# vshmyhlo/retinanet-tensorflow

Hardware: AMD Instinct MI355X
Metric: train images/sec (MobileNetV2-FPN RetinaNet 512x512, bs=2/GPU) (higher is better)
Workload: dtype f32

## Files before the change

include/rn_hip.h:

```cpp
#ifndef RN_HIP_H
#define RN_HIP_H

#include <stddef.h>
#include <stdint.h>

#ifdef __cplusplus
extern "C" {
#endif

typedef void* rn_stream_t;

enum rn_status {
  RN_OK = 0,
  RN_EINVAL = -1,
  RN_EUNSUPPORTED = -2,
  RN_EHIP = -3,
  RN_EWORKSPACE = -4
};

enum rn_act { RN_ACT_NONE = 0, RN_ACT_RELU = 1, RN_ACT_ELU = 2, RN_ACT_RELU6 = 3, RN_ACT_SIGMOID = 4 };
enum rn_loss_mode { RN_LOSS_BCE_DICE = 0, RN_LOSS_FOCAL = 1 };
enum rn_opt { RN_OPT_MOMENTUM = 0, RN_OPT_RMSPROP = 1, RN_OPT_ADAM = 2 };

#define RN_MAX_SEG 16

typedef struct rn_reduce_list rn_reduce_list;

#define RN_API_VERSION 411
int rn_version(void);
const char* rn_last_error(void);

void rn_same_pad(int n, int k, int s, int* out, int* pad_before);

typedef struct rn_conv_seg {
  const float* x;
  const float* wgt;
  const float* bias;
  float* y;
  const float* dy;
  float* dx;
  int32_t n, h, w;
  int32_t cout;
  int32_t x_ld;
// ... 252 lines not shown
typedef struct rn_wino_gn {
  const float* in_rows;
  const float* in_gamma;
  const float* in_beta;
  int32_t in_groups, in_act;
  float in_eps;
  float* out_rows;
  int32_t out_groups;
  const void* u_ready;
  int32_t urot_ready;
} rn_wino_gn;
size_t rn_wino_gn_rows(const rn_conv_seg* segs, int nseg, int tile);
size_t rn_conv3x3_winograd_gn_u_bytes(int cin, int cout, int tile);
int rn_conv3x3_winograd_gn_weights(const float* w, int cin, int cout, int tile, void* u_out, size_t u_out_bytes, float* urot_out,
                                   rn_stream_t stream);
int rn_conv3x3_winograd_gn(const rn_conv_seg* segs, int nseg, int cin, int cout, const float* w, const float* bias, int tile,
                           const rn_wino_gn* gn, void* workspace, size_t workspace_bytes, float* v_buf, float* urot_buf,
                           rn_stream_t stream);
typedef struct rn_wino_gn_bwd {
  const float* in_rows;
  const float* in_gamma;
  const float* in_beta;
  int32_t in_groups, in_act;
  float in_eps;
  float* in_g_rows_group;
  float* in_g_rows_chan;
  const float* out_rows;
  const float* out_g_rows_group;
  const float* out_gamma;
  int32_t out_groups;
  float out_eps;
  int32_t defer_wgrad;
} rn_wino_gn_bwd;
int rn_conv3x3_winograd_gn_bwd(const rn_conv_seg* segs, int nseg, int cin, int cout, const float* w, float* dw, int accumulate,
                               int tile, const rn_wino_gn_bwd* gn, void* workspace, size_t workspace_bytes, const float* v_buf,
                               const float* urot_buf, rn_stream_t stream);
int rn_conv3x3_winograd_gn_bwd_wgrad(const rn_conv_seg* segs, int nseg, int cin, int cout, float* dw, int accumulate, int tile,
                                     void* workspace, size_t workspace_bytes, const float* v_buf, int urot_was_given, rn_stream_t stream);
int rn_reduce_rows(const float* in, float* out, int64_t count, int nrows, int accumulate, rn_stream_t stream, rn_reduce_list* defer);

typedef struct rn_mb_rows {
  float* rows;
  int32_t rows_per_sample, width, bn;
} rn_mb_rows;

typedef struct rn_mb_norm {
  const float* y;
  rn_mb_rows stat;
  float* mean; float* rstd;
  const float* gamma; const float* beta;
  int32_t c, groups, act;
  float eps, drop_rate;
  uint64_t drop_seed; const uint64_t* drop_seed_dev;
// ... 151 lines not shown
```

retinanet-tensorflow_amd/_rn.py:

```python
import ctypes as C
import os

import torch

_HERE = os.path.dirname(os.path.abspath(__file__))
LIB_PATH = os.environ.get("RN_LIB_PATH") or os.path.join(_HERE, "librn_hip.so")

MAX_SEG = 16
ACT = {None: 0, "none": 0, "linear": 0, "relu": 1, "elu": 2, "relu6": 3, "sigmoid": 4}
LOSS_MODE = {"bce_dice": 0, "focal": 1}
OPT = {"momentum": 0, "rmsprop": 1, "adam": 2}
OPT_BLOCK = 1024
LR_MAX_BOUNDARIES = 8
LOSS_STATS_HEADER = 8
API_VERSION = 411


class RnError(RuntimeError):
    pass


class LrSchedule(C.Structure):
    _fields_ = [("kind", C.c_int32), ("n_boundaries", C.c_int32), ("base_lr", C.c_double), ("warmup_factor", C.c_double),
                ("final_factor", C.c_double), ("decay_factor", C.c_double), ("warmup_steps", C.c_int64), ("total_steps", C.c_int64),
                ("boundaries", C.c_int64 * LR_MAX_BOUNDARIES)]


class ConvSeg(C.Structure):
    _fields_ = [("x", C.c_void_p), ("wgt", C.c_void_p), ("bias", C.c_void_p), ("y", C.c_void_p),
                ("dy", C.c_void_p), ("dx", C.c_void_p),
# ... 10 lines not shown
    _fields_ = [("kh", C.c_int32), ("kw", C.c_int32), ("stride", C.c_int32), ("cin", C.c_int32),
                ("groups", C.c_int32)]


class WinoGn(C.Structure):
    _fields_ = [("in_rows", C.c_void_p), ("in_gamma", C.c_void_p), ("in_beta", C.c_void_p), ("in_groups", C.c_int32),
                ("in_act", C.c_int32), ("in_eps", C.c_float), ("out_rows", C.c_void_p), ("out_groups", C.c_int32),
                ("u_ready", C.c_void_p), ("urot_ready", C.c_int32)]


class WinoGnBwd(C.Structure):
    _fields_ = [("in_rows", C.c_void_p), ("in_gamma", C.c_void_p), ("in_beta", C.c_void_p), ("in_groups", C.c_int32),
                ("in_act", C.c_int32), ("in_eps", C.c_float), ("in_g_rows_group", C.c_void_p), ("in_g_rows_chan", C.c_void_p),
                ("out_rows", C.c_void_p), ("out_g_rows_group", C.c_void_p), ("out_gamma", C.c_void_p),
                ("out_groups", C.c_int32), ("out_eps", C.c_float), ("defer_wgrad", C.c_int32)]


class ReduceDesc(C.Structure):
    _fields_ = [("in_", C.c_void_p), ("out", C.c_void_p), ("count", C.c_int32), ("nrows", C.c_uint16), ("accumulate", C.c_uint16)]


class ReduceList(C.Structure):
    _fields_ = [("desc", C.POINTER(ReduceDesc)), ("capacity", C.c_int32), ("count", C.c_int32)]

    @classmethod
    def make(cls, capacity=1024):
        arr = (ReduceDesc * capacity)()
        lst = cls(C.cast(arr, C.POINTER(ReduceDesc)), capacity, 0)
        lst._keep = arr
        return lst
# ... 94 lines not shown
    "rn_conv3x3_winograd_bwd_workspace", "rn_conv3x3_winograd_bwd", "rn_flush_reductions", "rn_gemm_batched",
    "rn_winograd_bwd_products_workspace", "rn_winograd_bwd_products", "rn_wino_gn_rows", "rn_conv3x3_winograd_gn", "rn_conv3x3_winograd_gn_bwd", "rn_conv3x3_winograd_gn_bwd_wgrad", "rn_reduce_rows", "rn_resize_bilinear_normalize", "rn_resize_pair_u8",
    "rn_resize_pair_u8_augment_workspace", "rn_resize_pair_u8_augment",
    "rn_resize_pair_u8_batch", "rn_resize_pair_u8_augment_batch_workspace", "rn_resize_pair_u8_augment_batch",
    "rn_dwgn_supported", "rn_dwgn_fwd", "rn_dwgn_bwd", "rn_depthwise_fwd", "rn_depthwise_dgrad", "rn_depthwise_wgrad_workspace", "rn_depthwise_wgrad", "rn_depthwise_bwd",
    "rn_group_norm_sync_bytes", "rn_group_norm_workspace", "rn_group_norm_fwd", "rn_group_norm_bwd",
    "rn_act_fwd", "rn_act_bwd", "rn_upsample_add_fwd", "rn_upsample_add_bwd_top",
    "rn_pack_weights_f16", "rn_pack_weights_f16_bytes", "rn_cast_f32_to_f16", "rn_pad_cast_rgb_f16", "rn_conv2d_fwd_f16", "rn_conv2d_f16_fold_rows", "rn_conv2d_fwd_f16_fold", "rn_group_norm_finalize", "rn_group_norm_apply_f16", "rn_group_norm_apply_res_f16", "rn_maxpool_fwd_f16", "rn_maxpool_gn_fwd_f16", "rn_upsample_add_fwd_f16",
    "rn_act_fwd_f16", "rn_flip_width", "rn_dropout", "rn_dropout_strided", "rn_maxpool_fwd", "rn_maxpool_bwd", "rn_maxpool_bwd_arg", "rn_avgpool_fwd", "rn_avgpool_bwd",
    "rn_loss_workspace", "rn_loss_fwd", "rn_loss_bwd",
    "rn_iou", "rn_anchor_assign", "rn_anchor_assign_levels", "rn_anchor_assign_levels_pair", "rn_decode_boxes", "rn_detect_workspace", "rn_detect",
    "rn_boxes_decode", "rn_nms_classwise_workspace", "rn_nms_classwise",
    "rn_optimizer_workspace", "rn_grad_norm_l2reg", "rn_optimizer_step", "rn_counter_add", "rn_add_segs",
    "rn_mb_rows_max", "rn_mb_compact_rows_layout", "rn_mb_compact_rows", "rn_mb_pointwise_rows", "rn_mb_pointwise_fwd", "rn_mb_depthwise_rows", "rn_mb_depthwise_fwd", "rn_mb_apply",
    "rn_mb_resident_sync_bytes", "rn_mb_resident_rows", "rn_mb_resident_fwd", "rn_set_product_mode", "rn_get_product_mode",
    "rn_set_x3_bfrag", "rn_get_x3_bfrag", "rn_x3_bfrag_ok", "rn_x3_bfrag_bytes", "rn_x3_pack_bfrag", "rn_gemm_batched_bfrag", "rn_conv3x3_winograd_gn_u_bytes", "rn_conv3x3_winograd_gn_weights",
    "rn_conv2d_f16_stats_tiles", "rn_group_norm_fwd_f16_tiles",
    "rn_mb_pointwise_bwd_rows", "rn_mb_pointwise_bwd_workspace", "rn_mb_pointwise_bwd",
    "rn_mb_depthwise_bwd_rows", "rn_mb_depthwise_bwd_workspace", "rn_mb_depthwise_bwd",
    "rn_debug_collective_standin", "rn_optimizer_norm_pairs", "rn_optimizer_step_norm", "rn_norm_reg_finalize",
    "rn_lr_schedule_eval", "rn_optimizer_step_norm_lrdev",
]


def lib():
    global _lib
    if _lib is None:
        if not os.path.exists(LIB_PATH):
            raise RnError("librn_hip.so not found at %s: build it with "
                          "`make -C retinanet-tensorflow_amd/csrc` (there is no fallback path)" % LIB_PATH)
        L = C.CDLL(LIB_PATH)
# ... 68 lines not shown
        L.rn_conv3x3_winograd_bwd_workspace.argtypes = [C.c_void_p] + [C.c_int] * 6
        L.rn_conv3x3_winograd_bwd.argtypes = [C.c_void_p, C.c_int, C.c_int, C.c_int, C.c_void_p, C.c_void_p, C.c_int, C.c_int,
                                              C.c_void_p, C.c_size_t, C.c_void_p, C.c_void_p, C.c_void_p]
        L.rn_conv3x3_winograd_keep_bytes.argtypes = [C.c_void_p, C.c_int, C.c_int, C.c_int, C.c_int, C.c_void_p, C.c_void_p]
        L.rn_conv3x3_winograd.argtypes = [C.c_void_p, C.c_int, C.c_int, C.c_int, C.c_void_p, C.c_void_p, C.c_int, C.c_int,
                                          C.c_void_p, C.c_size_t, C.c_void_p, C.c_void_p, C.c_void_p]
        L.rn_wino_gn_rows.argtypes = [C.c_void_p, C.c_int, C.c_int]
        L.rn_winograd_bwd_products_workspace.argtypes = [C.c_int] * 4
        L.rn_winograd_bwd_products.argtypes = [C.c_void_p] * 3 + [C.c_int] * 3 + [C.c_void_p] * 2 + [C.c_int] * 3 + \
                                              [C.c_void_p, C.c_size_t, C.c_void_p, C.c_void_p]
        L.rn_x3_bfrag_ok.argtypes = [C.c_int] * 3
        L.rn_conv2d_f16_stats_tiles.argtypes = [C.c_void_p, C.c_int, C.c_void_p, C.c_void_p]
        L.rn_group_norm_fwd_f16_tiles.argtypes = [C.c_void_p, C.c_int, C.c_void_p, C.c_void_p, C.c_void_p, C.c_void_p, C.c_void_p, C.c_void_p]
        L.rn_conv3x3_winograd_gn_u_bytes.argtypes = [C.c_int] * 3
        L.rn_conv3x3_winograd_gn_weights.argtypes = [C.c_void_p, C.c_int, C.c_int, C.c_int, C.c_void_p, C.c_size_t, C.c_void_p, C.c_void_p]
        L.rn_x3_bfrag_bytes.argtypes = [C.c_int] * 3
        L.rn_x3_pack_bfrag.argtypes = [C.c_void_p, C.c_void_p] + [C.c_int] * 4 + [C.c_void_p]
        L.rn_gemm_batched_bfrag.argtypes = [C.c_void_p] * 3 + [C.c_int] * 5 + [C.c_void_p]
        L.rn_set_x3_bfrag.argtypes = [C.c_int]
        L.rn_conv3x3_winograd_gn.argtypes = [C.c_void_p, C.c_int, C.c_int, C.c_int, C.c_void_p, C.c_void_p, C.c_int, C.c_void_p,
                                             C.c_void_p, C.c_size_t, C.c_void_p, C.c_void_p, C.c_void_p]
        L.rn_conv3x3_winograd_gn_bwd_wgrad.argtypes = [C.c_void_p, C.c_int, C.c_int, C.c_int, C.c_void_p, C.c_int, C.c_int, C.c_void_p, C.c_size_t,
                                                       C.c_void_p, C.c_int, C.c_void_p]
        L.rn_conv3x3_winograd_gn_bwd.argtypes = [C.c_void_p, C.c_int, C.c_int, C.c_int, C.c_void_p, C.c_void_p, C.c_int, C.c_int,
                                                 C.c_void_p, C.c_void_p, C.c_size_t, C.c_void_p, C.c_void_p, C.c_void_p]
        L.rn_reduce_rows.argtypes = [C.c_void_p, C.c_void_p, C.c_int64, C.c_int, C.c_int, C.c_void_p, C.c_void_p]
        L.rn_conv2d_bias_grad.argtypes = [C.c_void_p, C.c_int, C.c_void_p, C.c_void_p, C.c_void_p, C.c_size_t,
                                          C.c_void_p, C.c_void_p]
        L.rn_group_norm_workspace.argtypes = [C.c_void_p, C.c_int, C.c_void_p]
        L.rn_group_norm_fwd.argtypes = [C.c_void_p, C.c_int, C.c_void_p, C.c_void_p, C.c_void_p, C.c_void_p,
                                        C.c_size_t, C.c_void_p]
        L.rn_group_norm_bwd.argtypes = [C.c_void_p, C.c_int, C.c_void_p, C.c_void_p, C.c_void_p, C.c_void_p,
                                        C.c_void_p, C.c_void_p, C.c_size_t, C.c_void_p, C.c_void_p]
        L.rn_act_fwd.argtypes = [C.c_void_p, C.c_void_p, C.c_int64, C.c_int, C.c_void_p]
        L.rn_act_bwd.argtypes = [C.c_void_p, C.c_void_p, C.c_void_p, C.c_int64, C.c_int, C.c_void_p]
        L.rn_upsample_add_fwd.argtypes = [C.c_void_p] * 3 + [C.c_int] * 6 + [C.c_void_p]
        L.rn_upsample_add_bwd_top.argtypes = [C.c_void_p] * 2 + [C.c_int] * 6 + [C.c_void_p]
        L.rn_pack_weights_f16.argtypes = [C.c_void_p, C.c_void_p, C.c_int, C.c_int, C.c_int, C.c_int, C.c_void_p]
# ... 225 lines not shown
```

retinanet-tensorflow_amd/csrc/winograd.hip:

```cpp
#include "rn_common.h"

namespace {
constexpr int NT = 256;

struct WSeg { const float* x; float* y; int n, h, w, th, tw, tile_start; };
struct WArgs {
  WSeg seg[RN_MAX_SEG];
  int nseg, c, total_tiles;
  float* buf;
  const float* bias;
};

__device__ __forceinline__ int seg_of_tile(const WArgs& a, int t) {
  int s = 0;
  while (s + 1 < a.nseg && t >= a.seg[s + 1].tile_start) ++s;
  return s;
}

template <int W>
struct VecW { typedef float type __attribute__((ext_vector_type(W))); };
template <>
struct VecW<1> { typedef float type; };

template <int M>
// ... 332 lines not shown
__host__ __device__ inline int weight_blocks_f32(const WeightArgs& wa) { return (wa.u || wa.u2) ? (int)((wa.kn + NT - 1) / NT) : 0; }
__host__ __device__ inline int weight_blocks_frag(const WeightArgs& wa) {
  return wa.uf ? (int)(((int64_t)(wa.cin / 2) * ((wa.cout + 31) / 32) * 32 + NT - 1) / NT) : 0;
}
__host__ __device__ inline int weight_blocks(const WeightArgs& wa) { return weight_blocks_f32(wa) + weight_blocks_frag(wa); }
template <int M>
__device__ __forceinline__ void wino_weight_any_body(const WeightArgs& wa, int blk) {
  const int n0 = weight_blocks_f32(wa);
  if (blk < n0) wino_weight_body<M>(wa.w, wa.u, wa.u2, wa.kn, wa.rot, blk);
  else wino_weight_frag_body<M>(wa.w, wa.uf, wa.cin, wa.cout, blk - n0);
}

template <int M>
__global__ __launch_bounds__(NT) void wino_weight_any_kernel(const WeightArgs wa) {
  wino_weight_any_body<M>(wa, blockIdx.x);
}

template <int M>
__global__ __launch_bounds__(NT) void wino_dw_kernel(const float* __restrict__ du, float* __restrict__ dw, int64_t kn, int nsplit,
                                                    int accumulate) {
  wino_dw_body<M>(du, dw, kn, nsplit, accumulate, blockIdx.x);
}
template <int M>
__global__ __launch_bounds__(NT) void wino_weight_kernel(const float* __restrict__ w, float* __restrict__ u, float* __restrict__ u2,
                                                        int64_t kn, int rot) {
  wino_weight_body<M>(w, u, u2, kn, rot, blockIdx.x);
}

struct DwArgs2 { const float* du; float* dw; int64_t kn; int nsplit, accumulate; };

// ... 760 lines not shown
template <int M, int W, template <int> class LT>
__global__ __launch_bounds__(chunk_threads<W>()) void wino_gn_input_kernel(const CArgs in, const Fold f, int slabs) {
  chunk_input_body<M, W, LT>(in, f, blockIdx.x / slabs, blockIdx.x % slabs);
}
template <int M, int W>
__global__ __launch_bounds__(chunk_threads<W>()) void wino_gn_output_kernel(const CArgs out, const Fold f, int slabs) {
  chunk_output_body<M, W, 0>(out, f, blockIdx.x / slabs, blockIdx.x % slabs);
}
template <int M, int W, template <int> class LT>
__global__ __launch_bounds__(chunk_threads<W>(), chunk_waves<W>()) void wino_gn_bwd_pre_kernel(const CArgs dgrad_in, const CArgs wgrad_dy, const Fold f,
                                                                               int nb_first, int slabs) {
  const int b = blockIdx.x;
  if (b < nb_first) chunk_input_body<M, W, LT>(dgrad_in, f, b / slabs, b % slabs);
  else chunk_dy_body<M, W, LT>(wgrad_dy, f, (b - nb_first) / slabs, (b - nb_first) % slabs);
}
template <int M, int W, int MODE>
__global__ __launch_bounds__(chunk_threads<W>(), chunk_waves<W>()) void wino_gn_bwd_post_kernel(const CArgs out, const Fold f, const DwArgs2 d, int nb_out,
                                                                                int slabs) {
  const int b = blockIdx.x;
  if (b < nb_out) chunk_output_body<M, W, MODE>(out, f, b / slabs, b % slabs);
  else wino_dw_body<M>(d.du, d.dw, d.kn, d.nsplit, d.accumulate, b - nb_out);
}

int cfill(const rn_conv_seg* segs, int nseg, int c, int m, CArgs* a, const float* const* xs, const float* const* auxs, float* const* ys) {
  int64_t tiles = 0, chunks = 0;
  for (int s = 0; s < nseg; ++s) {
    CSeg& d = a->seg[s];
    d.n = segs[s].n; d.h = segs[s].h; d.w = segs[s].w;
    d.th = (d.h + m - 1) / m; d.tw = (d.w + m - 1) / m;
    d.tile_start = (int)tiles; d.chunk_start = (int)chunks;
// ... 17 lines not shown
  return 2;
}
}

extern "C" size_t rn_wino_gn_rows(const rn_conv_seg* segs, int nseg, int tile) {
  if (!segs || nseg < 1 || nseg > RN_MAX_SEG || (tile != 2 && tile != 4)) return 0;
  size_t chunks = 0;
  for (int s = 0; s < nseg; ++s) {
    const size_t tps = (size_t)((segs[s].h + tile - 1) / tile) * ((segs[s].w + tile - 1) / tile);
    chunks += (size_t)segs[s].n * ((tps + CK_TILES - 1) / CK_TILES);
  }
  return chunks;
}

namespace {
#define RN_WGN(W_, CALL)                          \
  do {                                            \
    if (W_ == 4) { constexpr int W = 4; CALL; }   \
    else if (W_ == 2) { constexpr int W = 2; CALL; } \
    else { constexpr int W = 1; CALL; }           \
  } while (0)

template <int M>
int run_gn_fwd(const rn_conv_seg* segs, int nseg, int cin, int cout, const float* w, const float* bias, const rn_wino_gn* gn, float* U,
               float* V, float* Mb, float* v_buf, float* urot_buf, hipStream_t st) {
  constexpr int P2 = (M + 2) * (M + 2);
  const float* xs[RN_MAX_SEG]; float* ys[RN_MAX_SEG];
  for (int s = 0; s < nseg; ++s) { xs[s] = segs[s].x; ys[s] = segs[s].y; }
  CArgs ia = {}, oa = {};
  cfill(segs, nseg, cin, M, &ia, xs, nullptr, nullptr);
// ... 72 lines not shown
    fi.rows = gn->in_rows; fi.gamma = gn->in_gamma; fi.beta = gn->in_beta; fi.groups = gn->in_groups; fi.cpg = cin / gn->in_groups;
    fi.act = gn->in_act; fi.eps = gn->in_eps; fi.g_rows_group = gn->in_g_rows_group; fi.g_rows_chan = gn->in_g_rows_chan;
  }
  const int wi = chunk_width(T_, cin, fold_in ? fi.cpg : 0);
  if (!V) {
    CArgs xa = {};
    cfill(segs, nseg, cin, M, &xa, xins, nullptr, nullptr);
    xa.buf = (float*)(ws + L.v);
    const int slabs = cin / (CK_LANES * wi);
    if (fold_in) RN_WGN(wi, hipLaunchKernelGGL((wino_gn_input_kernel<M, W, LoadGnAct>), dim3(xa.total_chunks * slabs), dim3(chunk_threads<W>()), 0, st, xa, fi, slabs));
    else RN_WGN(wi, hipLaunchKernelGGL((wino_gn_input_kernel<M, W, LoadPlain>), dim3(xa.total_chunks * slabs), dim3(chunk_threads<W>()), 0, st, xa, fi, slabs));
    V = xa.buf;
  }
  ia.buf = Vdy;
  ya.buf = dM;
  if (fold_out) {
    Fold fo = {};
    fo.rows = gn->out_rows; fo.grows = gn->out_g_rows_group; fo.gamma = gn->out_gamma; fo.groups = gn->out_groups;
    fo.cpg = cout / gn->out_groups; fo.eps = gn->out_eps;
    const int wy = chunk_width(T_, cout, fo.cpg);
    const int slabs = cout / (CK_LANES * wy), nb = ia.total_chunks * slabs;
    RN_WGN(wy, hipLaunchKernelGGL((wino_gn_bwd_pre_kernel<M, W, LoadGnBwd>), dim3(2 * nb), dim3(chunk_threads<W>()), 0, st, ia, ya, fo, nb, slabs));
  } else {
    WArgs wia = {}, woa = {}, wya = {}, unused = {};
    if (int e = fill(segs, nseg, cin, cout, M, true, &wia, &woa, true)) return e;
    if (int e = fill(segs, nseg, cin, cout, M, true, &wya, &unused, true)) return e;
    wia.buf = Vdy; wya.buf = dM;
    const int wy = width_for(T_, cout);
    const int nb = (int)grid_for((int64_t)T_ * cout / wy);
    if (wy == 4) hipLaunchKernelGGL((wino_bwd_pre_kernel<M, 4>), dim3(2 * nb), dim3(NT), 0, st, wia, wya, nb);
    else if (wy == 2) hipLaunchKernelGGL((wino_bwd_pre_kernel<M, 2>), dim3(2 * nb), dim3(NT), 0, st, wia, wya, nb);
    else hipLaunchKernelGGL((wino_bwd_pre_kernel<M, 1>), dim3(2 * nb), dim3(NT), 0, st, wia, wya, nb);
  }
  RN_LAUNCH_CHECK();
  int nsplit = 1;
  const bool defer = gn->defer_wgrad != 0;
  if (defer) {
    if (int e = rn::launch_batched_gemm(Vdy, Urot, Mdx, T_, cout, cin, P2, 1, st)) return e;
  } else if (int e = rn::launch_winograd_bwd_products(Vdy, Urot, Mdx, T_, cout, cin, V, dM, cin, cout, P2, ws + L.slab, ws_bytes - L.slab, st,
                                                      &nsplit)) {
    return e;
  }
  oa.buf = Mdx; oa.bias = nullptr;
  {
    const DwArgs2 d = {(const float*)(ws + L.slab), dw, kn, nsplit, accumulate};
    const int slabs = cin / (CK_LANES * wi), nb_out = oa.total_chunks * slabs, nb_dw = defer ? 0 : (int)rn::ceil_div64(kn, NT);
    if (!fold_in) { fi.groups = 1; fi.cpg = CK_LANES * wi; }
    if (fold_in) RN_WGN(wi, hipLaunchKernelGGL((wino_gn_bwd_post_kernel<M, W, 1>), dim3(nb_out + nb_dw), dim3(chunk_threads<W>()), 0, st, oa, fi, d, nb_out, slabs));
    else RN_WGN(wi, hipLaunchKernelGGL((wino_gn_bwd_post_kernel<M, W, 0>), dim3(nb_out + nb_dw), dim3(chunk_threads<W>()), 0, st, oa, fi, d, nb_out, slabs));
  }
  RN_LAUNCH_CHECK();
  return RN_OK;
}
#undef RN_WGN

template <int M>
int run_gn_bwd_wgrad(const rn_conv_seg* segs, int nseg, int cin, int cout, float* dw, int accumulate, char* ws, const BwdLayout& L,
                     size_t ws_bytes, const float* v_buf, hipStream_t st) {
  constexpr int P2 = (M + 2) * (M + 2);
  const int T_ = (int)tiles_of(segs, nseg, M);
  const int64_t kn = (int64_t)cin * cout;
  const float* V = v_buf ? v_buf : (const float*)(ws + L.v);
  const float* dM = (const float*)(ws + L.dm);
  int nsplit = 1;
  if (int e = rn::launch_batched_gemm_tn(V, dM, nullptr, T_, cin, cout, P2, ws + L.slab, ws_bytes - L.slab, st, &nsplit, 1)) return e;
  hipLaunchKernelGGL(wino_dw_kernel<M>, dim3((unsigned)rn::ceil_div64(kn, NT)), dim3(NT), 0, st, (const float*)(ws + L.slab), dw, kn, nsplit,
                     accumulate);
  RN_LAUNCH_CHECK();
  return RN_OK;
}

int check_fold(const rn_conv_seg* segs, int nseg, int cin, int cout, int tile) {
  RN_CHECK_ARG(segs && nseg >= 1 && nseg <= RN_MAX_SEG && (tile == 2 || tile == 4), "winograd gn: bad segments / tile");
  RN_UNSUPPORTED(cin % CK_MAXCH != 0 || cout % 4 != 0, "winograd gn: cin %d must be a multiple of %d, cout %d of 4", cin, CK_MAXCH, cout);
  for (int s = 0; s < nseg; ++s) {
    RN_CHECK_ARG(segs[s].n >= 1 && segs[s].h >= 1 && segs[s].w >= 1, "winograd gn: bad segment %d", s);
    RN_UNSUPPORTED((double)segs[s].n * segs[s].h * segs[s].w * (cin > cout ? cin : cout) * 4.0 >= 2147483648.0,
                   "winograd gn: segment %d >= 2 GiB", s);
  }
  return RN_OK;
}
}

extern "C" size_t rn_conv3x3_winograd_gn_u_bytes(int cin, int cout, int tile) {
  if (cin < 1 || cout < 1 || (tile != 2 && tile != 4)) return 0;
  return u_bytes((size_t)(tile + 2) * (tile + 2), cin, cout);
}
extern "C" int rn_conv3x3_winograd_gn_weights(const float* w, int cin, int cout, int tile, void* u_out, size_t u_out_bytes, float* urot_out,
                                              rn_stream_t stream) {
  RN_CHECK_ARG(w && u_out && (tile == 2 || tile == 4), "winograd gn weights: bad argument");
  RN_UNSUPPORTED(cin % CK_MAXCH != 0 || cout % 4 != 0, "winograd gn weights: cin %d must be a multiple of %d, cout %d of 4", cin, CK_MAXCH, cout);
  const size_t need = rn_conv3x3_winograd_gn_u_bytes(cin, cout, tile);
  if (u_out_bytes < need) {
    rn::set_error("winograd gn weights: u_out %zu < %zu bytes", u_out_bytes, need);
    return RN_EWORKSPACE;
  }
  const bool u_frag = rn::x3_bfrag_format(cin, cout);
  const WeightArgs wa = {w, u_frag ? nullptr : (float*)u_out, urot_out, (int64_t)cin * cout, 0, u_frag ? (unsigned*)u_out : nullptr, cin, cout};
  hipStream_t st = (hipStream_t)stream;
  if (tile == 2) hipLaunchKernelGGL(wino_weight_any_kernel<2>, dim3((unsigned)weight_blocks(wa)), dim3(NT), 0, st, wa);
  else hipLaunchKernelGGL(wino_weight_any_kernel<4>, dim3((unsigned)weight_blocks(wa)), dim3(NT), 0, st, wa);
  RN_LAUNCH_CHECK();
  return RN_OK;
}

extern "C" int rn_conv3x3_winograd_gn_bwd_wgrad(const rn_conv_seg* segs, int nseg, int cin, int cout, float* dw, int accumulate, int tile,
                                                void* workspace, size_t workspace_bytes, const float* v_buf, int urot_was_given,
                                                rn_stream_t stream) {
  if (int e = check_fold(segs, nseg, cin, cout, tile)) return e;
  RN_CHECK_ARG(dw && workspace, "winograd gn bwd wgrad: null pointer");
  const BwdLayout L = bwd_layout(segs, nseg, cin, cout, tile, v_buf == nullptr, urot_was_given == 0);
  if (workspace_bytes < L.total) {
    rn::set_error("winograd gn bwd wgrad: workspace %zu < %zu bytes", workspace_bytes, L.total);
    return RN_EWORKSPACE;
  }
  hipStream_t st = (hipStream_t)stream;
  return tile == 2 ? run_gn_bwd_wgrad<2>(segs, nseg, cin, cout, dw, accumulate, (char*)workspace, L, workspace_bytes, v_buf, st)
                   : run_gn_bwd_wgrad<4>(segs, nseg, cin, cout, dw, accumulate, (char*)workspace, L, workspace_bytes, v_buf, st);
}

extern "C" int rn_conv3x3_winograd_gn(const rn_conv_seg* segs, int nseg, int cin, int cout, const float* w, const float* bias, int tile,
                                      const rn_wino_gn* gn, void* workspace, size_t workspace_bytes, float* v_buf, float* urot_buf,
                                      rn_stream_t stream) {
  if (int e = check_fold(segs, nseg, cin, cout, tile)) return e;
  RN_CHECK_ARG(w && workspace && gn, "winograd gn: null pointer");
  for (int s = 0; s < nseg; ++s) RN_CHECK_ARG(segs[s].x && segs[s].y, "winograd gn: null tensor in segment %d", s);
  if (gn->in_rows) {
    RN_CHECK_ARG(gn->in_gamma && gn->in_beta, "winograd gn: null gamma / beta");
    RN_UNSUPPORTED(!fold_ok(cin, gn->in_groups), "winograd gn: %d channels in %d groups cannot be folded", cin, gn->in_groups);
  }
  if (gn->out_rows) RN_UNSUPPORTED(!fold_ok(cout, gn->out_groups), "winograd gn: %d channels in %d groups cannot be folded", cout, gn->out_groups);
  const size_t need = rn_conv3x3_winograd_workspace(segs, nseg, cin, cout, tile);
  if (workspace_bytes < need) {
// ... 3 lines not shown
  const size_t p2 = (size_t)(tile + 2) * (tile + 2), tiles = tiles_of(segs, nseg, tile);
  RN_UNSUPPORTED((double)tiles * (cin > cout ? cin : cout) * 4.0 >= 2147483648.0, "winograd gn: a transform plane is >= 2 GiB");
  float* U = (float*)workspace;
  float* V = (float*)((char*)workspace + rn::align_up(u_bytes(p2, cin, cout), 256));
  float* Mb = (float*)((char*)V + rn::align_up(p2 * tiles * cin * 4, 256));
  hipStream_t st = (hipStream_t)stream;
  return tile == 2 ? run_gn_fwd<2>(segs, nseg, cin, cout, w, bias, gn, U, V, Mb, v_buf, urot_buf, st)
                   : run_gn_fwd<4>(segs, nseg, cin, cout, w, bias, gn, U, V, Mb, v_buf, urot_buf, st);
}

extern "C" int rn_conv3x3_winograd_gn_bwd(const rn_conv_seg* segs, int nseg, int cin, int cout, const float* w, float* dw, int accumulate,
                                          int tile, const rn_wino_gn_bwd* gn, void* workspace, size_t workspace_bytes, const float* v_buf,
                                          const float* urot_buf, rn_stream_t stream) {
  if (int e = check_fold(segs, nseg, cin, cout, tile)) return e;
  RN_CHECK_ARG(w && dw && workspace && gn, "winograd gn bwd: null pointer");
  for (int s = 0; s < nseg; ++s) RN_CHECK_ARG(segs[s].x && segs[s].dy && segs[s].dx, "winograd gn bwd: null tensor in segment %d", s);
  if (gn->in_rows) {
    RN_CHECK_ARG(gn->in_gamma && gn->in_beta && gn->in_g_rows_group && gn->in_g_rows_chan, "winograd gn bwd: null input-side pointer");
    RN_UNSUPPORTED(!fold_ok(cin, gn->in_groups), "winograd gn bwd: %d channels in %d groups cannot be folded", cin, gn->in_groups);
  }
  if (gn->out_rows) {
    RN_CHECK_ARG(gn->out_g_rows_group && gn->out_gamma, "winograd gn bwd: null output-side pointer");
    for (int s = 0; s < nseg; ++s) RN_CHECK_ARG(segs[s].y, "winograd gn bwd: the folded output side needs the raw conv output y (segment %d)", s);
    RN_UNSUPPORTED(!fold_ok(cout, gn->out_groups), "winograd gn bwd: %d channels in %d groups cannot be folded", cout, gn->out_groups);
  }
  const BwdLayout L = bwd_layout(segs, nseg, cin, cout, tile, v_buf == nullptr, urot_buf == nullptr);
  if (workspace_bytes < L.total) {
    rn::set_error("winograd gn bwd: workspace %zu < %zu bytes", workspace_bytes, L.total);
    return RN_EWORKSPACE;
  }
// ... 5 lines not shown
```

retinanet-tensorflow_amd/ops.py:

```python
import ctypes as C
import os

import torch

import _rn


DIRECT_PARAM_GRADS = False


WGRAD_SIDE_STREAM = False


class _on_side_stream(object):

    def __init__(self, device, tensors, direct=True):
        self.on = WGRAD_SIDE_STREAM and direct and device.type == 'cuda'
        if self.on:
            self.side = _rn.side_stream(device, 0)
            self.side.wait_stream(torch.cuda.current_stream(device))
            for t in tensors:
                if t is not None:
                    t.record_stream(self.side)
            self.ctx = torch.cuda.stream(self.side)
# ... 418 lines not shown
    for w, gamma, beta in tower:
        kh, kw, ci, co = w.shape
        g = gn_groups(co, groups)
        if not (kh == 3 and kw == 3 and ci == cin and ci % 64 == 0 and co % 64 == 0 and 64 % (co // g) == 0):
            return False
        cin = co
    if out_w is not None and not (out_w.shape[0] == 3 and out_w.shape[1] == 3 and out_w.shape[2] == cin and out_w.shape[3] % 4 == 0):
        return False
    m = WINOGRAD_TILE
    tiles = sum(x.shape[0] * ((x.shape[1] + m - 1) // m) * ((x.shape[2] + m - 1) // m) for x in xs)
    widest = max([cin] + [t[0].shape[3] for t in tower] + ([out_w.shape[3]] if out_w is not None else []))
    return 4 * (m + 2) ** 2 * (tiles * 2 * widest + widest * widest) <= WINOGRAD_MAX_WORKSPACE


WINO_PRE = {}


class WinoPretransform(object):

    def __init__(self, weights):
        L = _rn.lib()
        self.items = []
        for w in weights:
            cin, cout = int(w.shape[2]), int(w.shape[3])
            ub = int(L.rn_conv3x3_winograd_gn_u_bytes(cin, cout, WINOGRAD_TILE))
            u = torch.empty((ub + 3) // 4, dtype=torch.float32, device=w.device)
            urot = torch.empty((WINOGRAD_TILE + 2) ** 2 * cin * cout, dtype=torch.float32, device=w.device)
            self.items.append((w, u, urot))

    def launch(self):
        L = _rn.lib()
        for w, u, urot in self.items:
            _rn.check(L.rn_conv3x3_winograd_gn_weights(_rn.f32(w), int(w.shape[2]), int(w.shape[3]), WINOGRAD_TILE, u.data_ptr(), u.numel() * 4,
                                                       _rn.f32(urot), _rn.stream()), "rn_conv3x3_winograd_gn_weights")
        ev = torch.cuda.Event()
        ev.record(torch.cuda.current_stream())
        return {w.data_ptr(): (u, urot, ev) for w, u, urot in self.items}, ev


class _WinoTower(torch.autograd.Function):

    @staticmethod
    def forward(ctx, cfg, n, *args):
        groups, eps, act, k, with_out = cfg
        xs = [x.contiguous() for x in args[:n]]
        params = list(args[n:])
        tower = [(params[3 * i], params[3 * i + 1], params[3 * i + 2]) for i in range(k)]
        out_w, out_b = (params[3 * k], params[3 * k + 1]) if with_out else (None, None)
        L = _rn.lib()
# ... 87 lines not shown
                gnb.in_rows, gnb.in_gamma, gnb.in_beta = ctx.rows[i - 1].data_ptr(), _rn.f32(gamma), _rn.f32(beta)
                gnb.in_groups, gnb.in_act, gnb.in_eps = g_in, _rn.ACT[act], eps
                gnb.in_g_rows_group, gnb.in_g_rows_chan = grg.data_ptr(), grc.data_ptr()
            if i < nfold:
                _, gamma_o, _b = tower[i]
                for j in range(n):
                    segs[j].y = _rn.f32(inputs[i + 1][j])
                gnb.out_rows, gnb.out_g_rows_group = ctx.rows[i].data_ptr(), g_rows_group_next.data_ptr()
                gnb.out_gamma, gnb.out_groups, gnb.out_eps = _rn.f32(gamma_o), gn_groups(cout, groups), eps
            v_buf, u_buf = ctx.keep[i]
            dw_buf, dw = _grad_slot(w)
            need = L.rn_conv3x3_winograd_bwd_workspace(segs, n, cin, cout, tile, 1 if v_buf is not None else 0,
                                                       1 if u_buf is not None else 0)
            defer = WGRAD_DEFER is not None and dw is None
            ws = torch.empty(int(need), dtype=torch.uint8, device=dev) if defer else _rn.workspace(need, dev)
            gnb.defer_wgrad = 1 if defer else 0
            _rn.check(L.rn_conv3x3_winograd_gn_bwd(segs, n, cin, cout, _rn.f32(w), _rn.f32(dw_buf), 0, tile, C.byref(gnb),
                                                   ws.data_ptr(), ws.numel(),
                                                   _rn.f32(v_buf) if v_buf is not None else None,
                                                   _rn.f32(u_buf) if u_buf is not None else None, _rn.stream()),
                      "rn_conv3x3_winograd_gn_bwd")
            if defer:
                WGRAD_DEFER.append((segs, n, cin, cout, dw_buf, tile, ws, v_buf, 1 if u_buf is not None else 0, x_in))
            grads[3 * i if i < k else 3 * k] = dw
            if i == nconv - 1 and out_b is not None and ctx.needs_input_grad[2 + n + 3 * k + 1]:
                db_buf, db = _grad_slot(out_b)
                geom = _rn.ConvGeom(3, 3, 1, cin, 1)
                need = L.rn_conv2d_bias_grad_workspace(cout)
                wsb = _grad_workspace(need, dev)
                _rn.check(L.rn_conv2d_bias_grad(segs, n, C.byref(geom), _rn.f32(db_buf), wsb.data_ptr(), wsb.numel(), _rn.stream(), _defer_arg()),
                          "rn_conv2d_bias_grad")
                grads[3 * k + 1] = db
            if i > 0:
                _, gamma, beta = tower[i - 1]
                dg_buf, dg = _grad_slot(gamma)
                db_buf, db = _grad_slot(beta)
                if _deferring:
                    _deferred_keep.append(grc)
                _rn.check(L.rn_reduce_rows(_rn.f32(grc[0]), _rn.f32(db_buf), cin, ctx.nrows, 0, _rn.stream(), _defer_arg()), "rn_reduce_rows")
                _rn.check(L.rn_reduce_rows(_rn.f32(grc[1]), _rn.f32(dg_buf), cin, ctx.nrows, 0, _rn.stream(), _defer_arg()), "rn_reduce_rows")
                grads[3 * (i - 1) + 1], grads[3 * (i - 1) + 2] = dg, db
            cur_dy = dxs
            g_rows_group_next = grg
        return (None, None) + tuple(cur_dy) + tuple(grads)


WGRAD_DEFER = None


def run_deferred_wgrads(records):
    L = _rn.lib()
    for segs, n, cin, cout, dw_buf, tile, ws, v_buf, urot_given, _keep in records:
        _rn.check(L.rn_conv3x3_winograd_gn_bwd_wgrad(segs, n, cin, cout, _rn.f32(dw_buf), 0, tile, ws.data_ptr(), ws.numel(),
                                                     _rn.f32(v_buf) if v_buf is not None else None, urot_given, _rn.stream()),
                  "rn_conv3x3_winograd_gn_bwd_wgrad")


def wino_tower(xs, tower, out_w=None, out_b=None, groups=32, eps=1e-5, act=None):
    k = len(tower)
    cfg = (groups, float(eps), act, k, out_w is not None)
    flat = [t for layer in tower for t in layer]
    if out_w is not None:
        flat += [out_w, out_b]
    return list(_WinoTower.apply(cfg, len(xs), *xs, *flat))


class _Depthwise(torch.autograd.Function):

    @staticmethod
# ... 696 lines not shown
```

Measured before the change: 479.8.

## Batch winograd weight pretransforms into one launch; optionally defer dy transform to wgrad

New measurement: 480.5 (median of 3 runs). No clear change (+0.2%).

```diff
diff --git a/include/rn_hip.h b/include/rn_hip.h
--- a/include/rn_hip.h
+++ b/include/rn_hip.h
@@ -26,7 +26,7 @@
 
 typedef struct rn_reduce_list rn_reduce_list;
 
-#define RN_API_VERSION 411
+#define RN_API_VERSION 412
 int rn_version(void);
 const char* rn_last_error(void);
 
@@ -309,6 +309,15 @@
 size_t rn_conv3x3_winograd_gn_u_bytes(int cin, int cout, int tile);
 int rn_conv3x3_winograd_gn_weights(const float* w, int cin, int cout, int tile, void* u_out, size_t u_out_bytes, float* urot_out,
                                    rn_stream_t stream);
+#define RN_WINO_MAX_KERNELS 16
+typedef struct rn_wino_kernel {
+  const float* w;
+  int32_t cin, cout;
+  void* u_out;
+  size_t u_out_bytes;
+  float* urot_out;
+} rn_wino_kernel;
+int rn_conv3x3_winograd_gn_weights_many(const rn_wino_kernel* kernels, int nkernels, int tile, int max_blocks, rn_stream_t stream);
 int rn_conv3x3_winograd_gn(const rn_conv_seg* segs, int nseg, int cin, int cout, const float* w, const float* bias, int tile,
                            const rn_wino_gn* gn, void* workspace, size_t workspace_bytes, float* v_buf, float* urot_buf,
                            rn_stream_t stream);
@@ -331,7 +340,8 @@
                                int tile, const rn_wino_gn_bwd* gn, void* workspace, size_t workspace_bytes, const float* v_buf,
                                const float* urot_buf, rn_stream_t stream);
 int rn_conv3x3_winograd_gn_bwd_wgrad(const rn_conv_seg* segs, int nseg, int cin, int cout, float* dw, int accumulate, int tile,
-                                     void* workspace, size_t workspace_bytes, const float* v_buf, int urot_was_given, rn_stream_t stream);
+                                     void* workspace, size_t workspace_bytes, const float* v_buf, int urot_was_given,
+                                     const rn_wino_gn_bwd* gn, rn_stream_t stream);
 int rn_reduce_rows(const float* in, float* out, int64_t count, int nrows, int accumulate, rn_stream_t stream, rn_reduce_list* defer);
 
 typedef struct rn_mb_rows {
diff --git a/retinanet-tensorflow_amd/_rn.py b/retinanet-tensorflow_amd/_rn.py
--- a/retinanet-tensorflow_amd/_rn.py
+++ b/retinanet-tensorflow_amd/_rn.py
@@ -13,7 +13,7 @@
 OPT_BLOCK = 1024
 LR_MAX_BOUNDARIES = 8
 LOSS_STATS_HEADER = 8
-API_VERSION = 411
+API_VERSION = 412
 
 
 class RnError(RuntimeError):
@@ -54,6 +54,14 @@
                 ("in_act", C.c_int32), ("in_eps", C.c_float), ("in_g_rows_group", C.c_void_p), ("in_g_rows_chan", C.c_void_p),
                 ("out_rows", C.c_void_p), ("out_g_rows_group", C.c_void_p), ("out_gamma", C.c_void_p),
                 ("out_groups", C.c_int32), ("out_eps", C.c_float), ("defer_wgrad", C.c_int32)]
+
+
+WINO_MAX_KERNELS = 16
+
+
+class WinoKernel(C.Structure):
+    _fields_ = [("w", C.c_void_p), ("cin", C.c_int32), ("cout", C.c_int32), ("u_out", C.c_void_p), ("u_out_bytes", C.c_size_t),
+                ("urot_out", C.c_void_p)]
 
 
 class ReduceDesc(C.Structure):
@@ -178,7 +186,7 @@
     "rn_optimizer_workspace", "rn_grad_norm_l2reg", "rn_optimizer_step", "rn_counter_add", "rn_add_segs",
     "rn_mb_rows_max", "rn_mb_compact_rows_layout", "rn_mb_compact_rows", "rn_mb_pointwise_rows", "rn_mb_pointwise_fwd", "rn_mb_depthwise_rows", "rn_mb_depthwise_fwd", "rn_mb_apply",
     "rn_mb_resident_sync_bytes", "rn_mb_resident_rows", "rn_mb_resident_fwd", "rn_set_product_mode", "rn_get_product_mode",
-    "rn_set_x3_bfrag", "rn_get_x3_bfrag", "rn_x3_bfrag_ok", "rn_x3_bfrag_bytes", "rn_x3_pack_bfrag", "rn_gemm_batched_bfrag", "rn_conv3x3_winograd_gn_u_bytes", "rn_conv3x3_winograd_gn_weights",
+    "rn_set_x3_bfrag", "rn_get_x3_bfrag", "rn_x3_bfrag_ok", "rn_x3_bfrag_bytes", "rn_x3_pack_bfrag", "rn_gemm_batched_bfrag", "rn_conv3x3_winograd_gn_u_bytes", "rn_conv3x3_winograd_gn_weights", "rn_conv3x3_winograd_gn_weights_many",
     "rn_conv2d_f16_stats_tiles", "rn_group_norm_fwd_f16_tiles",
     "rn_mb_pointwise_bwd_rows", "rn_mb_pointwise_bwd_workspace", "rn_mb_pointwise_bwd",
     "rn_mb_depthwise_bwd_rows", "rn_mb_depthwise_bwd_workspace", "rn_mb_depthwise_bwd",
@@ -277,6 +285,7 @@
         L.rn_group_norm_fwd_f16_tiles.argtypes = [C.c_void_p, C.c_int, C.c_void_p, C.c_void_p, C.c_void_p, C.c_void_p, C.c_void_p, C.c_void_p]
         L.rn_conv3x3_winograd_gn_u_bytes.argtypes = [C.c_int] * 3
         L.rn_conv3x3_winograd_gn_weights.argtypes = [C.c_void_p, C.c_int, C.c_int, C.c_int, C.c_void_p, C.c_size_t, C.c_void_p, C.c_void_p]
+        L.rn_conv3x3_winograd_gn_weights_many.argtypes = [C.c_void_p, C.c_int, C.c_int, C.c_int, C.c_void_p]
         L.rn_x3_bfrag_bytes.argtypes = [C.c_int] * 3
         L.rn_x3_pack_bfrag.argtypes = [C.c_void_p, C.c_void_p] + [C.c_int] * 4 + [C.c_void_p]
         L.rn_gemm_batched_bfrag.argtypes = [C.c_void_p] * 3 + [C.c_int] * 5 + [C.c_void_p]
@@ -284,7 +293,7 @@
         L.rn_conv3x3_winograd_gn.argtypes = [C.c_void_p, C.c_int, C.c_int, C.c_int, C.c_void_p, C.c_void_p, C.c_int, C.c_void_p,
                                              C.c_void_p, C.c_size_t, C.c_void_p, C.c_void_p, C.c_void_p]
         L.rn_conv3x3_winograd_gn_bwd_wgrad.argtypes = [C.c_void_p, C.c_int, C.c_int, C.c_int, C.c_void_p, C.c_int, C.c_int, C.c_void_p, C.c_size_t,
-                                                       C.c_void_p, C.c_int, C.c_void_p]
+                                                       C.c_void_p, C.c_int, C.c_void_p, C.c_void_p]
         L.rn_conv3x3_winograd_gn_bwd.argtypes = [C.c_void_p, C.c_int, C.c_int, C.c_int, C.c_void_p, C.c_void_p, C.c_int, C.c_int,
                                                  C.c_void_p, C.c_void_p, C.c_size_t, C.c_void_p, C.c_void_p, C.c_void_p]
         L.rn_reduce_rows.argtypes = [C.c_void_p, C.c_void_p, C.c_int64, C.c_int, C.c_int, C.c_void_p, C.c_void_p]
diff --git a/retinanet-tensorflow_amd/csrc/winograd.hip b/retinanet-tensorflow_amd/csrc/winograd.hip
--- a/retinanet-tensorflow_amd/csrc/winograd.hip
+++ b/retinanet-tensorflow_amd/csrc/winograd.hip
@@ -370,6 +370,21 @@
 template <int M>
 __global__ __launch_bounds__(NT) void wino_weight_any_kernel(const WeightArgs wa) {
   wino_weight_any_body<M>(wa, blockIdx.x);
+}
+
+struct WeightManyArgs {
+  WeightArgs e[RN_WINO_MAX_KERNELS];
+  int start[RN_WINO_MAX_KERNELS + 1];
+  int n;
+};
+template <int M>
+__global__ __launch_bounds__(NT) void wino_weight_many_kernel(const WeightManyArgs a) {
+  const int total = a.start[a.n];
+  for (int b = (int)blockIdx.x; b < total; b += (int)gridDim.x) {
+    int e = 0;
+    while (e + 1 < a.n && b >= a.start[e + 1]) ++e;
+    wino_weight_any_body<M>(a.e[e], b - a.start[e]);
+  }
 }
 
 template <int M>
@@ -1160,6 +1175,10 @@
   if (b < nb_first) chunk_input_body<M, W, LT>(dgrad_in, f, b / slabs, b % slabs);
   else chunk_dy_body<M, W, LT>(wgrad_dy, f, (b - nb_first) / slabs, (b - nb_first) % slabs);
 }
+template <int M, int W, template <int> class LT>
+__global__ __launch_bounds__(chunk_threads<W>(), chunk_waves<W>()) void wino_gn_dy_kernel(const CArgs wgrad_dy, const Fold f, int slabs) {
+  chunk_dy_body<M, W, LT>(wgrad_dy, f, blockIdx.x / slabs, blockIdx.x % slabs);
+}
 template <int M, int W, int MODE>
 __global__ __launch_bounds__(chunk_threads<W>(), chunk_waves<W>()) void wino_gn_bwd_post_kernel(const CArgs out, const Fold f, const DwArgs2 d, int nb_out,
                                                                                 int slabs) {
@@ -1207,6 +1226,12 @@
 }
 
 namespace {
+Fold fold_out_side(const rn_wino_gn_bwd* gn, int cout) {
+  Fold fo = {};
+  fo.rows = gn->out_rows; fo.grows = gn->out_g_rows_group; fo.gamma = gn->out_gamma; fo.groups = gn->out_groups;
+  fo.cpg = cout / gn->out_groups; fo.eps = gn->out_eps;
+  return fo;
+}
 #define RN_WGN(W_, CALL)                          \
   do {                                            \
     if (W_ == 4) { constexpr int W = 4; CALL; }   \
@@ -1309,13 +1334,13 @@
   }
   ia.buf = Vdy;
   ya.buf = dM;
+  const bool defer = gn->defer_wgrad != 0;
+  const int halves = gn->defer_wgrad == 2 ? 1 : 2;
   if (fold_out) {
-    Fold fo = {};
-    fo.rows = gn->out_rows; fo.grows = gn->out_g_rows_group; fo.gamma = gn->out_gamma; fo.groups = gn->out_groups;
-    fo.cpg = cout / gn->out_groups; fo.eps = gn->out_eps;
+    const Fold fo = fold_out_side(gn, cout);
     const int wy = chunk_width(T_, cout, fo.cpg);
     const int slabs = cout / (CK_LANES * wy), nb = ia.total_chunks * slabs;
-    RN_WGN(wy, hipLaunchKernelGGL((wino_gn_bwd_pre_kernel<M, W, LoadGnBwd>), dim3(2 * nb), dim3(chunk_threads<W>()), 0, st, ia, ya, fo, nb, slabs));
+    RN_WGN(wy, hipLaunchKernelGGL((wino_gn_bwd_pre_kernel<M, W, LoadGnBwd>), dim3(halves * nb), dim3(chunk_threads<W>()), 0, st, ia, ya, fo, nb, slabs));
   } else {
     WArgs wia = {}, woa = {}, wya = {}, unused = {};
     if (int e = fill(segs, nseg, cin, cout, M, true, &wia, &woa, true)) return e;
@@ -1323,13 +1348,12 @@
     wia.buf = Vdy; wya.buf = dM;
     const int wy = width_for(T_, cout);
     const int nb = (int)grid_for((int64_t)T_ * cout / wy);
-    if (wy == 4) hipLaunchKernelGGL((wino_bwd_pre_kernel<M, 4>), dim3(2 * nb), dim3(NT), 0, st, wia, wya, nb);
-    else if (wy == 2) hipLaunchKernelGGL((wino_bwd_pre_kernel<M, 2>), dim3(2 * nb), dim3(NT), 0, st, wia, wya, nb);
-    else hipLaunchKernelGGL((wino_bwd_pre_kernel<M, 1>), dim3(2 * nb), dim3(NT), 0, st, wia, wya, nb);
+    if (wy == 4) hipLaunchKernelGGL((wino_bwd_pre_kernel<M, 4>), dim3(halves * nb), dim3(NT), 0, st, wia, wya, nb);
+    else if (wy == 2) hipLaunchKernelGGL((wino_bwd_pre_kernel<M, 2>), dim3(halves * nb), dim3(NT), 0, st, wia, wya, nb);
+    else hipLaunchKernelGGL((wino_bwd_pre_kernel<M, 1>), dim3(halves * nb), dim3(NT), 0, st, wia, wya, nb);
   }
   RN_LAUNCH_CHECK();
   int nsplit = 1;
-  const bool defer = gn->defer_wgrad != 0;
   if (defer) {
     if (int e = rn::launch_batched_gemm(Vdy, Urot, Mdx, T_, cout, cin, P2, 1, st)) return e;
   } else if (int e = rn::launch_winograd_bwd_products(Vdy, Urot, Mdx, T_, cout, cin, V, dM, cin, cout, P2, ws + L.slab, ws_bytes - L.slab, st,
@@ -1347,16 +1371,35 @@
   RN_LAUNCH_CHECK();
   return RN_OK;
 }
-#undef RN_WGN
 
 template <int M>
-int run_gn_bwd_wgrad(const rn_conv_seg* segs, int nseg, int cin, int cout, float* dw, int accumulate, char* ws, const BwdLayout& L,
-                     size_t ws_bytes, const float* v_buf, hipStream_t st) {
+int run_gn_bwd_wgrad(const rn_conv_seg* segs, int nseg, int cin, int cout, float* dw, int accumulate, const rn_wino_gn_bwd* gn, char* ws,
+                     const BwdLayout& L, size_t ws_bytes, const float* v_buf, hipStream_t st) {
   constexpr int P2 = (M + 2) * (M + 2);
   const int T_ = (int)tiles_of(segs, nseg, M);
   const int64_t kn = (int64_t)cin * cout;
   const float* V = v_buf ? v_buf : (const float*)(ws + L.v);
   const float* dM = (const float*)(ws + L.dm);
+  if (gn && gn->defer_wgrad == 2) {
+    if (gn->out_rows) {
+      const float* dys[RN_MAX_SEG]; const float* youts[RN_MAX_SEG];
+      for (int s = 0; s < nseg; ++s) { dys[s] = segs[s].dy; youts[s] = segs[s].y; }
+      CArgs ya = {};
+      cfill(segs, nseg, cout, M, &ya, dys, youts, nullptr);
+      ya.buf = (float*)(ws + L.dm);
+      const Fold fo = fold_out_side(gn, cout);
+      const int wy = chunk_width(T_, cout, fo.cpg);
+      const int slabs = cout / (CK_LANES * wy), nb = ya.total_chunks * slabs;
+      RN_WGN(wy, hipLaunchKernelGGL((wino_gn_dy_kernel<M, W, LoadGnBwd>), dim3(nb), dim3(chunk_threads<W>()), 0, st, ya, fo, slabs));
+    } else {
+      WArgs wya = {}, unused = {};
+      if (int e = fill(segs, nseg, cin, cout, M, true, &wya, &unused, true)) return e;
+      wya.buf = (float*)(ws + L.dm);
+      const int wy = width_for(T_, cout);
+      RN_WINO_LAUNCH(wino_dy_kernel, wy, (int64_t)T_ * cout, wya);
+    }
+    RN_LAUNCH_CHECK();
+  }
   int nsplit = 1;
   if (int e = rn::launch_batched_gemm_tn(V, dM, nullptr, T_, cin, cout, P2, ws + L.slab, ws_bytes - L.slab, st, &nsplit, 1)) return e;
   hipLaunchKernelGGL(wino_dw_kernel<M>, dim3((unsigned)rn::ceil_div64(kn, NT)), dim3(NT), 0, st, (const float*)(ws + L.slab), dw, kn, nsplit,
@@ -1364,6 +1407,7 @@
   RN_LAUNCH_CHECK();
   return RN_OK;
 }
+#undef RN_WGN
 
 int check_fold(const rn_conv_seg* segs, int nseg, int cin, int cout, int tile) {
   RN_CHECK_ARG(segs && nseg >= 1 && nseg <= RN_MAX_SEG && (tile == 2 || tile == 4), "winograd gn: bad segments / tile");
@@ -1381,8 +1425,8 @@
   if (cin < 1 || cout < 1 || (tile != 2 && tile != 4)) return 0;
   return u_bytes((size_t)(tile + 2) * (tile + 2), cin, cout);
 }
-extern "C" int rn_conv3x3_winograd_gn_weights(const float* w, int cin, int cout, int tile, void* u_out, size_t u_out_bytes, float* urot_out,
-                                              rn_stream_t stream) {
+namespace {
+int weight_entry(const float* w, int cin, int cout, int tile, void* u_out, size_t u_out_bytes, float* urot_out, WeightArgs* wa) {
   RN_CHECK_ARG(w && u_out && (tile == 2 || tile == 4), "winograd gn weights: bad argument");
   RN_UNSUPPORTED(cin % CK_MAXCH != 0 || cout % 4 != 0, "winograd gn weights: cin %d must be a multiple of %d, cout %d of 4", cin, CK_MAXCH, cout);
   const size_t need = rn_conv3x3_winograd_gn_u_bytes(cin, cout, tile);
@@ -1391,27 +1435,63 @@
     return RN_EWORKSPACE;
   }
   const bool u_frag = rn::x3_bfrag_format(cin, cout);
-  const WeightArgs wa = {w, u_frag ? nullptr : (float*)u_out, urot_out, (int64_t)cin * cout, 0, u_frag ? (unsigned*)u_out : nullptr, cin, cout};
+  *wa = WeightArgs{w, u_frag ? nullptr : (float*)u_out, urot_out, (int64_t)cin * cout, 0, u_frag ? (unsigned*)u_out : nullptr, cin, cout};
+  return RN_OK;
+}
+}
+extern "C" int rn_conv3x3_winograd_gn_weights(const float* w, int cin, int cout, int tile, void* u_out, size_t u_out_bytes, float* urot_out,
+                                              rn_stream_t stream) {
+  WeightArgs wa;
+  if (int e = weight_entry(w, cin, cout, tile, u_out, u_out_bytes, urot_out, &wa)) return e;
   hipStream_t st = (hipStream_t)stream;
   if (tile == 2) hipLaunchKernelGGL(wino_weight_any_kernel<2>, dim3((unsigned)weight_blocks(wa)), dim3(NT), 0, st, wa);
   else hipLaunchKernelGGL(wino_weight_any_kernel<4>, dim3((unsigned)weight_blocks(wa)), dim3(NT), 0, st, wa);
   RN_LAUNCH_CHECK();
   return RN_OK;
 }
+extern "C" int rn_conv3x3_winograd_gn_weights_many(const rn_wino_kernel* kernels, int nkernels, int tile, int max_blocks, rn_stream_t stream) {
+  RN_CHECK_ARG(kernels && nkernels >= 1 && nkernels <= RN_WINO_MAX_KERNELS, "winograd gn weights: %d kernels (1 .. %d)", nkernels,
+               RN_WINO_MAX_KERNELS);
+  WeightManyArgs a = {};
+  int64_t total = 0;
+  for (int i = 0; i < nkernels; ++i) {
+    const rn_wino_kernel& k = kernels[i];
+    if (int e = weight_entry(k.w, k.cin, k.cout, tile, k.u_out, k.u_out_bytes, k.urot_out, &a.e[i])) return e;
+    a.start[i] = (int)total;
+    total += weight_blocks(a.e[i]);
+    RN_UNSUPPORTED(total >= 2147483647, "winograd gn weights: too many blocks");
+  }
+  a.start[nkernels] = (int)total;
+  a.n = nkernels;
+  const unsigned grid = (unsigned)(max_blocks > 0 && max_blocks < total ? max_blocks : total);
+  hipStream_t st = (hipStream_t)stream;
+  if (tile == 2) hipLaunchKernelGGL(wino_weight_many_kernel<2>, dim3(grid), dim3(NT), 0, st, a);
+  else hipLaunchKernelGGL(wino_weight_many_kernel<4>, dim3(grid), dim3(NT), 0, st, a);
+  RN_LAUNCH_CHECK();
+  return RN_OK;
+}
 
 extern "C" int rn_conv3x3_winograd_gn_bwd_wgrad(const rn_conv_seg* segs, int nseg, int cin, int cout, float* dw, int accumulate, int tile,
                                                 void* workspace, size_t workspace_bytes, const float* v_buf, int urot_was_given,
-                                                rn_stream_t stream) {
+                                                const rn_wino_gn_bwd* gn, rn_stream_t stream) {
   if (int e = check_fold(segs, nseg, cin, cout, tile)) return e;
   RN_CHECK_ARG(dw && workspace, "winograd gn bwd wgrad: null pointer");
+  if (gn && gn->defer_wgrad == 2) {
+    for (int s = 0; s < nseg; ++s) RN_CHECK_ARG(segs[s].dy, "winograd gn bwd wgrad: null dy in segment %d", s);
+    if (gn->out_rows) {
+      RN_CHECK_ARG(gn->out_g_rows_group && gn->out_gamma, "winograd gn bwd wgrad: null output-side pointer");
+      for (int s = 0; s < nseg; ++s) RN_CHECK_ARG(segs[s].y, "winograd gn bwd wgrad: the folded output side needs the raw conv output y (segment %d)", s);
+      RN_UNSUPPORTED(!fold_ok(cout, gn->out_groups), "winograd gn bwd wgrad: %d channels in %d groups cannot be folded", cout, gn->out_groups);
+    }
+  }
   const BwdLayout L = bwd_layout(segs, nseg, cin, cout, tile, v_buf == nullptr, urot_was_given == 0);
   if (workspace_bytes < L.total) {
     rn::set_error("winograd gn bwd wgrad: workspace %zu < %zu bytes", workspace_bytes, L.total);
     return RN_EWORKSPACE;
   }
   hipStream_t st = (hipStream_t)stream;
-  return tile == 2 ? run_gn_bwd_wgrad<2>(segs, nseg, cin, cout, dw, accumulate, (char*)workspace, L, workspace_bytes, v_buf, st)
-                   : run_gn_bwd_wgrad<4>(segs, nseg, cin, cout, dw, accumulate, (char*)workspace, L, workspace_bytes, v_buf, st);
+  return tile == 2 ? run_gn_bwd_wgrad<2>(segs, nseg, cin, cout, dw, accumulate, gn, (char*)workspace, L, workspace_bytes, v_buf, st)
+                   : run_gn_bwd_wgrad<4>(segs, nseg, cin, cout, dw, accumulate, gn, (char*)workspace, L, workspace_bytes, v_buf, st);
 }
 
 extern "C" int rn_conv3x3_winograd_gn(const rn_conv_seg* segs, int nseg, int cin, int cout, const float* w, const float* bias, int tile,
@@ -1445,6 +1525,7 @@
                                           const float* urot_buf, rn_stream_t stream) {
   if (int e = check_fold(segs, nseg, cin, cout, tile)) return e;
   RN_CHECK_ARG(w && dw && workspace && gn, "winograd gn bwd: null pointer");
+  RN_CHECK_ARG(gn->defer_wgrad >= 0 && gn->defer_wgrad <= 2, "winograd gn bwd: defer_wgrad %d (0, 1 or 2)", gn->defer_wgrad);
   for (int s = 0; s < nseg; ++s) RN_CHECK_ARG(segs[s].x && segs[s].dy && segs[s].dx, "winograd gn bwd: null tensor in segment %d", s);
   if (gn->in_rows) {
     RN_CHECK_ARG(gn->in_gamma && gn->in_beta && gn->in_g_rows_group && gn->in_g_rows_chan, "winograd gn bwd: null input-side pointer");
diff --git a/retinanet-tensorflow_amd/ops.py b/retinanet-tensorflow_amd/ops.py
--- a/retinanet-tensorflow_amd/ops.py
+++ b/retinanet-tensorflow_amd/ops.py
@@ -456,6 +456,7 @@
 
 
 WINO_PRE = {}
+WINO_PRE_BLOCKS = int(os.environ.get("RN_WINO_PRE_BLOCKS", "256"))
 
 
 class WinoPretransform(object):
@@ -469,12 +470,19 @@
             u = torch.empty((ub + 3) // 4, dtype=torch.float32, device=w.device)
             urot = torch.empty((WINOGRAD_TILE + 2) ** 2 * cin * cout, dtype=torch.float32, device=w.device)
             self.items.append((w, u, urot))
-
-    def launch(self):
-        L = _rn.lib()
-        for w, u, urot in self.items:
-            _rn.check(L.rn_conv3x3_winograd_gn_weights(_rn.f32(w), int(w.shape[2]), int(w.shape[3]), WINOGRAD_TILE, u.data_ptr(), u.numel() * 4,
-                                                       _rn.f32(urot), _rn.stream()), "rn_conv3x3_winograd_gn_weights")
+        assert 1 <= len(self.items) <= _rn.WINO_MAX_KERNELS, "rn_conv3x3_winograd_gn_weights_many takes 1 .. %d kernels" % _rn.WINO_MAX_KERNELS
+        self.table = (_rn.WinoKernel * len(self.items))()
+        for e, (w, u, urot) in zip(self.table, self.items):
+            e.w, e.cin, e.cout = _rn.f32(w), int(w.shape[2]), int(w.shape[3])
+            e.u_out, e.u_out_bytes, e.urot_out = u.data_ptr(), u.numel() * 4, _rn.f32(urot)
+
+    def launch(self, max_blocks=None):
+        L = _rn.lib()
+        for e, (w, _u, _urot) in zip(self.table, self.items):
+            e.w = _rn.f32(w)
+        _rn.check(L.rn_conv3x3_winograd_gn_weights_many(self.table, len(self.items), WINOGRAD_TILE,
+                                                        WINO_PRE_BLOCKS if max_blocks is None else int(max_blocks), _rn.stream()),
+                  "rn_conv3x3_winograd_gn_weights_many")
         ev = torch.cuda.Event()
         ev.record(torch.cuda.current_stream())
         return {w.data_ptr(): (u, urot, ev) for w, u, urot in self.items}, ev
@@ -592,14 +600,16 @@
                                                        1 if u_buf is not None else 0)
             defer = WGRAD_DEFER is not None and dw is None
             ws = torch.empty(int(need), dtype=torch.uint8, device=dev) if defer else _rn.workspace(need, dev)
-            gnb.defer_wgrad = 1 if defer else 0
+            gnb.defer_wgrad = (2 if WGRAD_DEFER_DY else 1) if defer else 0
             _rn.check(L.rn_conv3x3_winograd_gn_bwd(segs, n, cin, cout, _rn.f32(w), _rn.f32(dw_buf), 0, tile, C.byref(gnb),
                                                    ws.data_ptr(), ws.numel(),
                                                    _rn.f32(v_buf) if v_buf is not None else None,
                                                    _rn.f32(u_buf) if u_buf is not None else None, _rn.stream()),
                       "rn_conv3x3_winograd_gn_bwd")
             if defer:
-                WGRAD_DEFER.append((segs, n, cin, cout, dw_buf, tile, ws, v_buf, 1 if u_buf is not None else 0, x_in))
+                keep = (x_in, cur_dy, inputs[i + 1] if i < nfold else None, ctx.rows[i] if i < nfold else None, g_rows_group_next)
+                WGRAD_DEFER.append((segs, n, cin, cout, dw_buf, tile, ws, v_buf, 1 if u_buf is not None else 0,
+                                    gnb if gnb.defer_wgrad == 2 else None, keep))
             grads[3 * i if i < k else 3 * k] = dw
             if i == nconv - 1 and out_b is not None and ctx.needs_input_grad[2 + n + 3 * k + 1]:
                 db_buf, db = _grad_slot(out_b)
@@ -624,13 +634,15 @@
 
 
 WGRAD_DEFER = None
+WGRAD_DEFER_DY = os.environ.get("RN_DEFER_DY", "0") == "1"
 
 
 def run_deferred_wgrads(records):
     L = _rn.lib()
-    for segs, n, cin, cout, dw_buf, tile, ws, v_buf, urot_given, _keep in records:
+    for segs, n, cin, cout, dw_buf, tile, ws, v_buf, urot_given, gnb, _keep in records:
         _rn.check(L.rn_conv3x3_winograd_gn_bwd_wgrad(segs, n, cin, cout, _rn.f32(dw_buf), 0, tile, ws.data_ptr(), ws.numel(),
-                                                     _rn.f32(v_buf) if v_buf is not None else None, urot_given, _rn.stream()),
+                                                     _rn.f32(v_buf) if v_buf is not None else None, urot_given,
+                                                     C.byref(gnb) if gnb is not None else None, _rn.stream()),
                   "rn_conv3x3_winograd_gn_bwd_wgrad")
 
 
```
